# fabriceo/AVDSP

Hardware: AMD Instinct MI355X
Metric: Msamples/s (all ch) biquad+FIR chain (higher is better)
Workload: dtype f64; 1 GPU; north: 4096 ch x (16 biquads + 4096-tap FIR), block 1024 frames, DSP_FORMAT 6; 4096 ch in total, 4096 ch/GPU by dspRuntimeSetShard(rank, 1), no data-path collective; channels=4096, channels_per_gpu=4096, taps=4096, block=1024, format=6, overlap=1, ready_words=-1, ready_mode=2, side_by_side=1, streams_remade=0, cu_split=0, fir_split=0, fir_launch=-1, fir_lean=-1, ring_wait=1

## Files before the change

avdsp_amd/csrc/avdsp_host.c:

```c
#include "avdsp_runtime.h"
#include "avdsp_hip.h"

#include <stdarg.h>
#include <stdio.h>
#include <stdlib.h>
#include <string.h>

dspHeader_t *dspHeaderPtr = 0;
int          dspBiquadFreqSkip = 0;
int          dspMantissa = DSP_MANT;

const char *dspOpcodeText[DSP_MAX_OPCODE] = {
    "DSP_END_OF_CODE", "\nDSP_HEADER", "DSP_NOP", "\nDSP_CORE", "\nDSP_PARAM", "\nDSP_PARAM_NUM",
    "DSP_SERIAL", "DSP_TPDF_CALC", "DSP_TPDF", "DSP_WHITE", "DSP_CLRXY", "DSP_SWAPXY", "DSP_COPYXY",
    "DSP_COPYYX", "DSP_ADDXY", "DSP_ADDYX", "DSP_SUBXY", "DSP_SUBYX", "DSP_MULXY", "DSP_DIVXY",
    "DSP_DIVYX", "DSP_AVGXY", "DSP_AVGYX", "DSP_NEGX", "DSP_NEGY", "DSP_SQRTX", "DSP_SHIFT",
    "DSP_VALUE", "DSP_VALUE_INT", "DSP_MUL_VALUE", "DSP_MUL_VALUE_INT", "DSP_DIV_VALUE",
    "DSP_DIV_VALUE_INT", "DSP_AND_VALUE_INT", "DSP_LOAD", "DSP_LOAD_GAIN", "DSP_LOAD_MUX",
    "DSP_STORE", "DSP_LOAD_STORE", "DSP_LOAD_MEM", "DSP_STORE_MEM", "DSP_GAIN", "DSP_SAT0DB",
    "DSP_SAT0DB_TPDF", "DSP_SAT0DB_GAIN", "DSP_SAT0DB_TPDF_GAIN", "DSP_DELAY_1", "DSP_DELAY",
    "DSP_DELAY_DP", "DSP_DATA_TABLE", "DSP_BIQUADS", "DSP_FIR", "DSP_RMS", "DSP_DCBLOCK",
    "DSP_DITHER", "DSP_DITHER_NS2", "DSP_DISTRIB", "DSP_DIRAC", "DSP_SQUAREWAVE", "DSP_CLIP",
    "DSP_LOAD_MEM_DATA", "DSP_SINE"
};
// ... 52 lines not shown
    int             biquad_freq_skip, mantissa;
    int             device_ordinal;
    int             ninst;
    int             inst_saved_lanes;
    int             inst_saved_generic;
    int             inst_call;
    size_t          inst_in_words, inst_out_words;
    int             opt_cu_split;
    int             opt_group_serial;
    int             inst_chain_mode;
    int             chain_inst_made;
    size_t          chain_inst_in, chain_inst_out;
    int             chain_inst_win[5];
    int             opt_frame_server, opt_frame_server_idle_us;
    int             opt_fir_shared;
} avdsp_ctx;

static avdsp_ctx g_template = { .opt_lane_hw = 1, .opt_ring_wait = 1, .opt_ready_words = -1, .opt_fir_impl = 1, .opt_biquad_impl = 1, .opt_device = -1, .opt_interp_impl = 1, .opt_strand_split = 1, .opt_strand_lanes = 1, .shard_world = 1,
                                .mantissa = DSP_MANT, .device_ordinal = -1, .opt_frame_server_idle_us = 1000, .opt_fir_shared = 1 };

__attribute__((constructor)) static void frame_server_from_environment(void)
{
    const char *e = getenv("AVDSP_FRAME_SERVER");
    if (e && !strcmp(e, "1")) g_template.opt_frame_server = 1;
}
#define MAX_PROGRAMS 64
static avdsp_ctx *g_ctx[MAX_PROGRAMS];
static int        g_nctx;
static avdsp_ctx *g_cur = &g_template;
#define G (*g_cur)
static int        g_rate_static;

static char g_err[512];
static int  g_err_code;
static int  ensure_encoding(int format);

static int fail(int code, const char *fmt, ...)
{
    va_list ap;
// ... 130 lines not shown
        G.opt_host_pin = value;
        return 0;
    }
    if (!strcmp(key, "fir_lean")) {
        if (G.dev && avdsp_hip_prog_set_option(G.dev, AVDSP_OPT_FIR_LEAN, value)) return hip_fail();
        G.opt_fir_lean = value; G.opt_fir_lean_set = 1;
        return 0;
    }
    if (!strcmp(key, "fir_shared")) {
        if (value != 0 && value != 1) return fail(-1, "fir_shared: 0 or 1");
        if (G.dev && avdsp_hip_prog_set_option(G.dev, AVDSP_OPT_FIR_SHARED, value)) return hip_fail();
        G.opt_fir_shared = value;
        return 0;
    }
    if (!strcmp(key, "fir_shared_chains") || !strcmp(key, "fir_shared_groups")) return fail(-1, "%s is read-only", key);
    if (!strcmp(key, "ring_wait")) {
        if (G.dev && avdsp_hip_prog_set_option(G.dev, AVDSP_OPT_RING_WAIT, value)) return hip_fail();
        G.opt_ring_wait = value != 0;
        return 0;
    }
    if (!strcmp(key, "fir_launch")) {
        if (G.dev && avdsp_hip_prog_set_option(G.dev, AVDSP_OPT_FIR_LAUNCH, value)) return hip_fail();
        G.opt_fir_launch = value; G.opt_fir_launch_set = 1;
        return 0;
    }
    if (!strcmp(key, "profile_stride")) {
        if (value < 1) return fail(-1, "profile_stride: every n-th launch, n >= 1");
        if (G.dev && avdsp_hip_prog_set_option(G.dev, AVDSP_OPT_PROFILE_STRIDE, value)) return hip_fail();
        G.opt_profile_stride = value;
        return 0;
// ... 59 lines not shown
    if (!strcmp(key, "interp_impl")) return G.opt_interp_impl;
    if (!strcmp(key, "levels"))      return G.last_levels;
    if (!strcmp(key, "cores"))       return G.last_cores;
    if (!strcmp(key, "pieces"))      return G.last_pieces;
    if (!strcmp(key, "strand_split")) return G.opt_strand_split;
    if (!strcmp(key, "strand_lanes")) return G.opt_strand_lanes;
    if (!strcmp(key, "strands"))     return G.last_strands;
    if (!strcmp(key, "overlap"))     return G.opt_overlap;
    if (!strcmp(key, "ready_words")) return G.opt_ready_words;
    if (!strcmp(key, "lane_hw"))     return G.opt_lane_hw;
    if (!strcmp(key, "fir_split"))   return G.opt_fir_split;
    if (!strcmp(key, "fir_launch"))  return G.opt_fir_launch_set ? G.opt_fir_launch : -1;
    if (!strcmp(key, "fir_lean"))    return G.opt_fir_lean_set ? G.opt_fir_lean : -1;
    if (!strcmp(key, "ring_wait"))   return G.opt_ring_wait;
    if (!strcmp(key, "fir_shared"))  return G.opt_fir_shared;
    if (!strcmp(key, "fir_shared_chains")) { device_current(); return G.dev ? avdsp_hip_prog_get_option(G.dev, AVDSP_OPT_FIR_SHARED_CHAINS) : 0; }
    if (!strcmp(key, "fir_shared_groups")) { device_current(); return G.dev ? avdsp_hip_prog_get_option(G.dev, AVDSP_OPT_FIR_SHARED_GROUPS) : 0; }
    if (!strncmp(key, "timing_pairs_", 13) && key[13] >= '0' && key[13] <= '7' && !key[14])
        return G.dev ? avdsp_hip_profile_last_pairs(G.dev, key[13] - '0') : 0;
    if (!strcmp(key, "ready_timeouts")) { device_current(); return G.dev ? avdsp_hip_ready_timeouts(G.dev) : 0; }
    if (!strcmp(key, "cu_split"))    return G.opt_cu_split;
    if (!strcmp(key, "group_fanout")) return !G.opt_group_serial;
    if (!strcmp(key, "side_by_side")) { device_current(); return G.dev ? avdsp_hip_prog_get_option(G.dev, AVDSP_OPT_SIDE_BY_SIDE) : -1; }
    if (!strcmp(key, "streams_remade")) { device_current(); return G.dev ? avdsp_hip_prog_get_option(G.dev, AVDSP_OPT_STREAMS_REMADE) : 0; }
    if (!strcmp(key, "ready_mode"))  { device_current(); return G.dev ? avdsp_hip_prog_get_option(G.dev, AVDSP_OPT_READY_MODE) : 0; }
    if (!strcmp(key, "frame_server")) return G.opt_frame_server;
    if (!strcmp(key, "frame_server_idle_us")) return G.opt_frame_server_idle_us;
    if (!strcmp(key, "frame_server_frames")) return G.dev ? avdsp_hip_prog_get_option(G.dev, AVDSP_OPT_FRAME_SERVER_FRAMES) : 0;
    if (!strcmp(key, "frame_server_launches")) return G.dev ? avdsp_hip_prog_get_option(G.dev, AVDSP_OPT_FRAME_SERVER_LAUNCHES) : 0;
    if (!strcmp(key, "frame_server_fallbacks")) return G.dev ? avdsp_hip_prog_get_option(G.dev, AVDSP_OPT_FRAME_SERVER_FALLBACKS) : 0;
// ... 91 lines not shown
        const dspHeader_t *h = (const dspHeader_t *)codePtr;
        const opcode_t *lo = codePtr, *hi = codePtr + (long long)h->totalLength + (h->dataSize > 0 ? h->dataSize : 0);
        for (int i = 0; i < g_nctx; )
            if (g_ctx[i] != c && g_ctx[i]->code < hi && lo < g_ctx[i]->code + (g_ctx[i]->total_words > 0 ? g_ctx[i]->total_words : 1)) ctx_destroy(g_ctx[i]);
            else i++;
    }
    int fresh = 0;
    if (!c) {
        if (g_nctx == MAX_PROGRAMS) return fail(-9, "%d programs are loaded already: dspRuntimeReleaseProgram() the ones no longer used", MAX_PROGRAMS);
        c = (avdsp_ctx *)calloc(1, sizeof *c);
        if (!c) return fail(-9, "out of memory");
        const avdsp_ctx *o = &g_template;
        c->opt_fir_impl = o->opt_fir_impl; c->opt_biquad_impl = o->opt_biquad_impl; c->opt_device = o->opt_device; c->opt_profile = o->opt_profile;
        c->opt_generic = o->opt_generic; c->opt_interp_impl = o->opt_interp_impl; c->opt_strand_split = o->opt_strand_split; c->opt_strand_lanes = o->opt_strand_lanes;
        c->opt_profile_stride = o->opt_profile_stride; c->opt_overlap = o->opt_overlap; c->opt_fir_rows = o->opt_fir_rows; c->opt_host_split = o->opt_host_split; c->opt_host_pin = o->opt_host_pin; c->opt_ready_words = o->opt_ready_words; c->opt_lane_hw = o->opt_lane_hw; c->opt_fir_split = o->opt_fir_split; c->opt_fir_launch = o->opt_fir_launch; c->opt_fir_launch_set = o->opt_fir_launch_set; c->opt_fir_lean = o->opt_fir_lean; c->opt_fir_lean_set = o->opt_fir_lean_set; c->opt_ring_wait = o->opt_ring_wait; c->opt_cu_split = o->opt_cu_split; c->opt_group_serial = o->opt_group_serial;
        c->opt_frame_server = o->opt_frame_server; c->opt_frame_server_idle_us = o->opt_frame_server_idle_us; c->opt_fir_shared = o->opt_fir_shared;
        c->shard_rank = o->shard_rank; c->shard_world = o->shard_world;
        c->mantissa = DSP_MANT; c->device_ordinal = -1;
        c->code = codePtr;
        g_ctx[g_nctx++] = c;
        fresh = 1;
    }
    ctx_make_current(c);
    drop_device();
    G.have_rate = 0;
    dspHeaderPtr = (dspHeader_t *)codePtr;
    G.code = codePtr;
    G.total_words = 0;
#define INIT_FAIL(...) do { const int r_ = fail(__VA_ARGS__); if (fresh) { ctx_destroy(c); for (int i_ = 0; i_ < g_nctx; i_++) if (g_ctx[i_] == prev) ctx_make_current(prev); } return r_; } while (0)
    if (codePtr->op.opcode != DSP_HEADER) INIT_FAIL(-1, "no dsp header in this program");
    int length = dspHeaderPtr->totalLength, size = dspHeaderPtr->dataSize;
// ... 698 lines not shown
    if (!G.dev) return hip_fail();
    if (avdsp_hip_upload_words(G.dev, (const int32_t *)G.code, 0, G.total_words) ||
        avdsp_hip_tpdf_reset(G.dev, G.random, G.dither)) {
        hip_fail(); drop_device(); return g_err_code;
    }
    G.dev_state_valid = 1;
    avdsp_hip_profile_enable(G.dev, G.opt_profile);
    if (avdsp_hip_prog_set_option(G.dev, AVDSP_OPT_PROFILE_STRIDE, G.opt_profile_stride > 0 ? G.opt_profile_stride : 1) ||
        avdsp_hip_prog_set_option(G.dev, AVDSP_OPT_OVERLAP, G.opt_overlap) || avdsp_hip_prog_set_option(G.dev, AVDSP_OPT_FIR_ROWS, G.opt_fir_rows) ||
        avdsp_hip_prog_set_option(G.dev, AVDSP_OPT_READY_WORDS, G.opt_ready_words) || avdsp_hip_prog_set_option(G.dev, AVDSP_OPT_LANE_HW, G.opt_lane_hw) || avdsp_hip_prog_set_option(G.dev, AVDSP_OPT_FIR_SPLIT, G.opt_fir_split) || (G.opt_fir_launch_set && avdsp_hip_prog_set_option(G.dev, AVDSP_OPT_FIR_LAUNCH, G.opt_fir_launch)) || (G.opt_fir_lean_set && avdsp_hip_prog_set_option(G.dev, AVDSP_OPT_FIR_LEAN, G.opt_fir_lean)) || avdsp_hip_prog_set_option(G.dev, AVDSP_OPT_RING_WAIT, G.opt_ring_wait) ||
        avdsp_hip_prog_set_option(G.dev, AVDSP_OPT_HOST_SPLIT, G.opt_host_split) || avdsp_hip_prog_set_option(G.dev, AVDSP_OPT_HOST_PIN, G.opt_host_pin) ||
        (G.opt_cu_split && avdsp_hip_prog_set_option(G.dev, AVDSP_OPT_CU_SPLIT, G.opt_cu_split)) ||
        (G.opt_group_serial && avdsp_hip_prog_set_option(G.dev, AVDSP_OPT_GROUP_FANOUT, 0)) ||
        (G.opt_frame_server && avdsp_hip_prog_set_option(G.dev, AVDSP_OPT_FRAME_SERVER, 1)) ||
        (!G.opt_fir_shared && avdsp_hip_prog_set_option(G.dev, AVDSP_OPT_FIR_SHARED, 0)) ||
        (G.opt_frame_server_idle_us != 1000 && avdsp_hip_prog_set_option(G.dev, AVDSP_OPT_FRAME_SERVER_IDLE_US, G.opt_frame_server_idle_us)) ||
        (G.ninst > 1 && avdsp_hip_set_instances(G.dev, G.ninst))) {
        hip_fail(); drop_device(); return g_err_code;
    }
    return 0;
}

static const avdsp_chain *g_fg_chains;
static int fir_group_cmp(const void *pa, const void *pb)
{
    const avdsp_chain *a = &g_fg_chains[*(const int32_t *)pa], *b = &g_fg_chains[*(const int32_t *)pb];
    if (a->fir_coef_word != b->fir_coef_word) return a->fir_coef_word < b->fir_coef_word ? -1 : 1;
    if (a->fir_taps != b->fir_taps) return a->fir_taps < b->fir_taps ? -1 : 1;
    return *(const int32_t *)pa < *(const int32_t *)pb ? -1 : *(const int32_t *)pa > *(const int32_t *)pb;
}
// ... 1179 lines not shown
```

avdsp_amd/csrc/avdsp_kernels.hip:

```cpp
#include <hip/hip_runtime.h>
#include <hip/hip_ext.h>
#include <atomic>
#include <chrono>
#include <mutex>
#include <thread>

#include <cstdarg>
#include <cstdio>
#include <cstring>
#include <type_traits>
#include <utility>
#include <vector>
#include <algorithm>

#include "avdsp_hip.h"
#include "avdsp_format.h"

namespace {

thread_local char g_err[512];
thread_local bool g_err_ready = false;

int set_err(const char *fmt, ...)
{
// ... 3213 lines not shown
    double *d_taps64 = nullptr; int pitch64 = 0;
    int n_sh_groups = 0, n_sh_chains = 0;
    int *d_sh_ids = nullptr;
    SharedTile *d_sh_tiles = nullptr; int n_sh_tiles = 0;
    double *d_sh_taps64 = nullptr;
    int *d_sh_feed = nullptr; int n_sh_feed = 0;
    int *d_fir_rest = nullptr; int n_fir_rest = 0;
    bool lane_mode = false;
    int *d_lane_rows = nullptr; int n_lane_rows = 0;
    int n_lane_feed = 0;
    int n_lane_fir = 0; unsigned *d_lseq = nullptr; int lseq_pitch = 0;
    avdsp_strand_op *d_sops = nullptr; int *d_sargs = nullptr; int s_nops = 0, s_nargs = 0, s_nstrands = 0, s_nres = 0; bool s_usey = false;
    std::vector<int> s_loaded, s_stored;
    bool stores_whole_window = false;
    bool overlap_ok = false;
    unsigned *d_ready = nullptr; unsigned seq = 0;
};

}

struct avdsp_hip_prog {
    int total_words = 0;
    int chain_inst = 0;
    int *d_buf = nullptr;
    TpdfGlobals *d_tpdf = nullptr;
    int *d_tpdf_seq = nullptr; int tpdf_seq_frames = 0;
    unsigned *d_frame = nullptr; int frame_words = 0;
    std::vector<Plan> plans;
    unsigned *d_in = nullptr, *d_out = nullptr; size_t in_cap = 0, out_cap = 0;
    struct Alias { hipStream_t stream; unsigned *buf; size_t cap; };
// ... 21 lines not shown
    std::vector<hipStream_t> side;
    std::vector<hipEvent_t> join;
    hipEvent_t fork = nullptr;
    int overlap = 0;
    int fir_rows = 0;
    int fir_lean = -1;
    int fir_split = 0;
    int fir_shared = 1;
    int sh_chains_now = 0, sh_groups_now = 0;
    hipStream_t s_bq = nullptr;
    hipStream_t s_fir[2] = {nullptr, nullptr};
    static constexpr int kAhead = 3;
    hipEvent_t ev_bq[kAhead] = {nullptr, nullptr, nullptr}, ev_fir[kAhead] = {nullptr, nullptr, nullptr};
    hipEvent_t ev_fir_now[kAhead] = {nullptr, nullptr, nullptr};
    hipEvent_t last_ride_stop = nullptr;
    int fir_launch_mode = -1, fir_mode_now = 0;
    hipEvent_t launch_ev[16] = {};
    unsigned launch_ev_next = 0;
    int lane_hw = 1;
    int ready_words = -1;
    int ready_mode_now = 0;
    int side_by_side = 0;
    std::vector<std::pair<hipStream_t, int>> probed;
    std::vector<hipStream_t> retired;
    int remade = 0;
    hipStream_t bq_side[3] = {nullptr, nullptr, nullptr};
    hipEvent_t bq_fork = nullptr, bq_join[3] = {nullptr, nullptr, nullptr};
    int group_fanout = 1;
    int cu_split = 0;
    unsigned *d_ready_timeouts = nullptr;
// ... 117 lines not shown
    if (v.empty()) return 0;
    HIP_TRY(hipMalloc((void **)dst, v.size() * sizeof(T)));
    return copy_from_caller(*dst, v.data(), v.size() * sizeof(T));
}

void free_plan(Plan &p)
{
    (void)hipFree(p.d_chains); (void)hipFree(p.d_sec_coef); (void)hipFree(p.d_sec_state);
    for (auto &g : p.bq) {
        (void)hipFree(g.d_ids); (void)hipFree(g.d_rows); (void)hipFree(g.d_lanes); (void)hipFree(g.d_scratch[0]); (void)hipFree(g.d_scratch[1]);
        for (auto &pc : g.pieces) { (void)hipFree(pc.d_ids); (void)hipFree(pc.d_rows); (void)hipFree(pc.d_lanes); }
    }
    (void)hipFree(p.d_rows_all); (void)hipFree(p.d_lanes_all);
    (void)hipFree(p.d_sops); (void)hipFree(p.d_sargs); (void)hipFree(p.d_lseq); (void)hipFree(p.d_lane_rows);
    (void)hipFree(p.d_fir_ids); (void)hipFree(p.d_pass_ids); (void)hipFree(p.d_ring); (void)hipFree(p.d_ring64); (void)hipFree(p.d_own); (void)hipFree(p.d_taps64);
    (void)hipFree(p.d_ready);
    (void)hipFree(p.d_sh_ids); (void)hipFree(p.d_sh_tiles); (void)hipFree(p.d_sh_taps64); (void)hipFree(p.d_sh_feed); (void)hipFree(p.d_fir_rest);
}

int fir_groups_per_chunk(int max_taps)
{
    const int G = (max_taps + 15 + 15) >> 4;
    const int nc = (G + kMaxGpc - 1) / kMaxGpc;
    const int gpc = (G + nc - 1) / nc;
    return std::min((gpc + kNG - 1) / kNG * kNG, kMaxGpc);
}

size_t fir_lds_bytes(int gpc, int *hs_cap, int *row)
{
    *hs_cap = (fir_hs_len(gpc) + 3) & ~3;
    *row = fir_win_row(gpc);
// ... 477 lines not shown
    HIP_TRY(hipEventRecord(prog->bq_fork, st));
    for (int k = 1; k < lanes; k++) HIP_TRY(hipStreamWaitEvent(prog->bq_side[k - 1], prog->bq_fork, 0));
    for (size_t gi = 0; gi < ng; gi++) {
        auto &g = *todo[gi];
        const int k = (int)(gi % (size_t)lanes);
        if (launch_group(g, k ? prog->bq_side[k - 1] : st, nullptr)) return -1;
    }
    for (int k = 1; k < lanes; k++) {
        HIP_TRY(hipEventRecord(prog->bq_join[k - 1], prog->bq_side[k - 1]));
        HIP_TRY(hipStreamWaitEvent(st, prog->bq_join[k - 1], 0));
    }
    if (last_stop) HIP_TRY(hipEventRecord(last_stop, st));
    return 0;
}

template <int FMT>
int launch_all(avdsp_hip_prog *prog, Plan &pl, BlockIO io, int fir_impl, int biquad_impl, hipStream_t stream)
{
    const bool under = prog->overlap && pl.overlap_ok && biquad_impl && fir_impl;
    pl.seq++;
    if (under) {
        prog->sh_chains_now = prog->sh_groups_now = 0;
        if (overlap_ready(prog)) return -1;
        const bool own_fir = prog->overlap >= 2 || prog->cu_split > 0;
        if (probe_side_by_side(prog, prog->overlap >= 2 ? prog->s_fir[prog->blk & 1] : prog->cu_split > 0 ? prog->s_fir[0] : stream)) return -1;
        const bool can_words = (fir_impl == 1 || fir_impl == 4) && pl.d_ready && prog->d_ready_timeouts && prog->side_by_side;
        const int rw = prog->ready_words >= 0 ? prog->ready_words : (prog->overlap == 1 && (long long)pl.n_fir * pl.max_taps >= 12000000ll ? 2 : 0);
        const bool behind = rw == 2 && can_words;
        const bool words = (rw == 1 && fir_impl == 1 && can_words) || behind;
        prog->ready_mode_now = behind ? 2 : words ? 1 : 0;
        const bool wt = words && !behind;
        const int slot = (int)(prog->blk % avdsp_hip_prog::kAhead);
        if (prog->ev_fir_set[slot]) {
            bool done = false;
            if (prog->ring_wait_host) {
                const auto t0 = std::chrono::steady_clock::now();
                for (;;) {
                    const hipError_t q = hipEventQuery(prog->ev_fir_now[slot]);
                    if (q == hipSuccess) { done = true; break; }
                    (void)hipGetLastError();
                    if (q != hipErrorNotReady) break;
                    if (std::chrono::steady_clock::now() - t0 > std::chrono::milliseconds(1)) break;
                    std::this_thread::yield();
                }
            }
            if (!done) HIP_TRY(hipStreamWaitEvent(prog->s_bq, prog->ev_fir_now[slot], 0));
        }
        if (prog->input_ready) HIP_TRY(hipStreamWaitEvent(prog->s_bq, prog->input_ready, 0));
        if (launch_cascades<FMT>(prog, pl, io, biquad_impl, prog->s_bq, !words ? prog->ev_bq[slot] : nullptr, wt)) return -1;
        if (behind && prog->ready_test > 0) prog->ready_test--;
        else if (behind) {
            hipLaunchKernelGGL(ready_set, dim3((unsigned)((pl.n_fir + kBlock - 1) / kBlock)), dim3(kBlock), 0, prog->s_bq, pl.d_ready, pl.d_fir_ids, pl.n_fir, pl.seq);
            HIP_TRY(hipGetLastError());
        }
        if (own_fir) {
            hipStream_t fs = prog->s_fir[prog->overlap >= 2 ? (prog->blk & 1) : 0];
            if (!words) HIP_TRY(hipStreamWaitEvent(fs, prog->ev_bq[slot], 0));
            if (launch_fir<FMT>(prog, pl, pl.d_fir_ids, pl.n_fir, io, fir_impl, fs, words)) return -1;
            HIP_TRY(hipEventRecord(prog->ev_fir[slot], fs));
            prog->ev_fir_now[slot] = prog->ev_fir[slot];
            HIP_TRY(hipStreamWaitEvent(stream, prog->ev_fir[slot], 0));
        } else {
            if (!words) HIP_TRY(hipStreamWaitEvent(stream, prog->ev_bq[slot], 0));
            const int mode = fir_impl != 1 && fir_impl != 4 ? 0 : prog->fir_launch_mode >= 0 ? prog->fir_launch_mode
                           : ((long long)pl.n_fir * pl.max_taps <= 6000000ll && io.nframes > 768) ? 2 : 1;
            const bool rides = mode == 1 && !((prog->profile >> AVDSP_KERNEL_FIR & 1u) && prog->profile_seen[AVDSP_KERNEL_FIR & 7] % (unsigned)prog->profile_stride == 0);
            prog->fir_mode_now = mode;
            prog->last_ride_stop = nullptr;
            const int rc_fir = launch_fir<FMT>(prog, pl, pl.d_fir_ids, pl.n_fir, io, fir_impl, stream, words, rides ? prog->ev_fir[slot] : nullptr);
            prog->fir_mode_now = 0;
            if (rc_fir) return -1;
            prog->ev_fir_now[slot] = prog->ev_fir[slot];
            static const bool timer_doubles = !getenv("AVDSP_TIMER_DOUBLES") || atoi(getenv("AVDSP_TIMER_DOUBLES")) != 0;
            if (!rides && mode == 1 && prog->last_ride_stop && timer_doubles) prog->ev_fir_now[slot] = prog->last_ride_stop;
            else if (!rides) HIP_TRY(hipEventRecord(prog->ev_fir[slot], stream));
        }
// ... 254 lines not shown
    (void)hipFree(p->d_tag_prev);
    for (auto &pn : p->pinned) if (pn.ours) (void)hipHostUnregister(const_cast<void *>(pn.ptr));
    for (auto st : {p->s_h2d, p->s_run, p->s_d2h}) if (st) (void)hipStreamDestroy(st);
    for (auto e : p->ev_host) (void)hipEventDestroy(e);
    for (auto st : {p->q_h2d, p->q_run, p->q_d2h}) if (st) { (void)hipStreamSynchronize(st); (void)hipStreamDestroy(st); }
    for (auto &sl : p->hq) {
        (void)hipFree(sl.d_in); (void)hipFree(sl.d_out);
        for (auto e : {sl.h2d, sl.run, sl.d2h}) if (e) (void)hipEventDestroy(e);
    }
    if (p->s_bq) (void)hipStreamDestroy(p->s_bq);
    for (auto st : p->retired) (void)hipStreamDestroy(st);
    for (auto st : p->bq_side) if (st) (void)hipStreamDestroy(st);
    for (auto e : p->bq_join) if (e) (void)hipEventDestroy(e);
    if (p->bq_fork) (void)hipEventDestroy(p->bq_fork);
    for (auto fs : p->s_fir) if (fs) (void)hipStreamDestroy(fs);
    if (p->ev_unpack) (void)hipEventDestroy(p->ev_unpack);
    for (int i = 0; i < avdsp_hip_prog::kAhead; i++) { if (p->ev_bq[i]) (void)hipEventDestroy(p->ev_bq[i]); if (p->ev_fir[i]) (void)hipEventDestroy(p->ev_fir[i]); }
    (void)hipFree(p->d_buf); (void)hipFree(p->d_in); (void)hipFree(p->d_out); (void)hipFree(p->d_tpdf); (void)hipFree(p->d_frame);
    (void)hipHostFree(p->h_small); (void)hipHostFree(p->h_ready_flag);
    (void)hipHostFree(p->fs_h); (void)hipFree(p->fs_table);
    for (auto e : p->launch_ev) if (e) (void)hipEventDestroy(e);
    (void)hipFree(p->d_tpdf_seq); (void)hipFree(p->d_ready_timeouts); for (auto &x : p->alias) (void)hipFree(x.buf);
    (void)hipFree(p->d_inst_buf); (void)hipFree(p->d_inst_tpdf); (void)hipFree(p->d_inst_frame); (void)hipFree(p->d_inst_seq);
    delete p;
}

int avdsp_hip_prog_add_plan(avdsp_hip_prog *prog, const avdsp_plan_desc *d)
{
    FS_STOP(prog);
    if (d->format < 2 || d->format > 6) return set_err("format %d has no device kernels", d->format);
// ... 115 lines not shown
            while (all_rows.size() % 4) { all_rows.push_back(empty); all_lanes.insert(all_lanes.end(), 16, LaneRec{-1, -1}); }
            pl.n_row_groups++;
            pl.rows_all_fir = pl.rows_all_fir && all_fir;
        }
        pl.bq.push_back(g);
    }
    if (upload_vec(&pl.d_chains, dev_chains)) { free_plan(pl); return -1; }
    if (pl.n_row_groups >= 2) {
        RowRec empty = all_rows.back(); empty.cid = -1;
        while (all_rows.size() % 16) { all_rows.push_back(empty); all_lanes.insert(all_lanes.end(), 16, LaneRec{-1, -1}); }
        pl.n_rows_all = (int)all_rows.size();
        if (upload_vec(&pl.d_rows_all, all_rows) || upload_vec(&pl.d_lanes_all, all_lanes)) { free_plan(pl); return -1; }
    }
    pl.n_fir = (int)fir.size(); pl.n_pass = (int)pass.size();
    if (upload_vec(&pl.d_fir_ids, fir) || upload_vec(&pl.d_pass_ids, pass)) { free_plan(pl); return -1; }
    if (pl.n_fir) {
        pl.fir_gpc = fir_groups_per_chunk(pl.max_taps);
        {
            int hs_cap, row;
            const int lds = (int)fir_lds_bytes(pl.fir_gpc, &hs_cap, &row);
            const void *variants[2] = { d->format == 4 ? (const void *)fir_mfma<4, 1> : (const void *)fir_mfma<6, 1>,
                                        d->format == 4 ? (const void *)fir_mfma<4, 2> : (const void *)fir_mfma<6, 2> };
            for (const void *fn : variants) {
                hipError_t e = hipFuncSetAttribute(fn, hipFuncAttributeMaxDynamicSharedMemorySize, lds);
                if (e != hipSuccess) { free_plan(pl); return set_err("hipFuncSetAttribute(LDS %d): %s", lds, hipGetErrorString(e)); }
            }
        }
        pl.ring_R = pow2ceil(pl.max_taps + avdsp_hip_prog::kAhead * kFirChunk + 16 * pl.fir_gpc + 16 * (kNG + 4) + 64);
        static_assert(kFirChunk == kFirPad, "one FIR launch covers exactly the frames the window image is laid out for");
        hipError_t e = hipMalloc((void **)&pl.d_ring, (size_t)d->nchains * 2 * pl.ring_R * sizeof(float));
// ... 1328 lines not shown
    (void)hipFree(d);
    return rc;
}

int avdsp_hip_prog_set_option(avdsp_hip_prog *prog, int key, int value)
{
    FS_STOP(prog);
    HIP_TRY(hipDeviceSynchronize());
    switch (key) {
    case AVDSP_OPT_OVERLAP:  prog->overlap = value; for (bool &f : prog->ev_fir_set) f = false; return 0;
    case AVDSP_OPT_READY_WORDS: if (value < -1 || value > 2) return set_err("ready_words: -1 (by plan), 0 (events), 1 (the cascade's waves publish) or 2 (a kernel behind the cascade publishes)"); prog->ready_words = value; return 0;
    case AVDSP_OPT_LANE_HW: prog->lane_hw = value != 0; return 0;
    case AVDSP_OPT_FIR_SPLIT: prog->fir_split = value != 0; return 0;
    case AVDSP_OPT_FIR_SHARED: if (value != 0 && value != 1) return set_err("fir_shared: 0 or 1"); prog->fir_shared = value; return 0;
    case AVDSP_OPT_FIR_LEAN: if (value < -1 || value > 1) return set_err("fir_lean: -1 (auto), 0 or 1"); prog->fir_lean = value; return 0;
    case AVDSP_OPT_RING_WAIT: prog->ring_wait_host = value != 0; return 0;
    case AVDSP_OPT_READY_TEST: prog->ready_test = value > 0 ? value : 0; return 0;
    case AVDSP_OPT_FRAME_SERVER: prog->fs_on = value != 0; return 0;
    case AVDSP_OPT_FRAME_SERVER_IDLE_US: if (value < 50 || value > 20000) return set_err("frame_server_idle_us: 50 .. 20000"); prog->fs_idle_us = value; return 0;
    case AVDSP_OPT_GROUP_FANOUT: prog->group_fanout = value != 0; return 0;
    case AVDSP_OPT_CU_SPLIT:
        if (value < -128 || value > 128 || (value & 7)) return set_err("cu_split: 0 (off) or 8, 16, ... 128 CUs for the cascades' stream (negative: the FIRs stay on the caller's stream, unmasked)");
        if (value != prog->cu_split) {
            if (prog->s_bq) { (void)hipStreamDestroy(prog->s_bq); prog->s_bq = nullptr; }
            for (auto &fs : prog->s_fir) if (fs) { (void)hipStreamDestroy(fs); fs = nullptr; }
            for (int i = 0; i < avdsp_hip_prog::kAhead; i++) {
                if (prog->ev_bq[i]) { (void)hipEventDestroy(prog->ev_bq[i]); prog->ev_bq[i] = nullptr; }
                if (prog->ev_fir[i]) { (void)hipEventDestroy(prog->ev_fir[i]); prog->ev_fir[i] = nullptr; }
                prog->ev_fir_set[i] = false; prog->ev_fir_now[i] = nullptr;
            }
// ... 19 lines not shown

int avdsp_hip_prog_get_option(avdsp_hip_prog *prog, int key)
{
    switch (key) {
    case AVDSP_OPT_SIDE_BY_SIDE: return prog->s_bq ? prog->side_by_side : -1;
    case AVDSP_OPT_READY_MODE:   return prog->ready_mode_now;
    case AVDSP_OPT_STREAMS_REMADE: return prog->remade;
    case AVDSP_OPT_FRAME_SERVER: return prog->fs_on;
    case AVDSP_OPT_FRAME_SERVER_IDLE_US: return prog->fs_idle_us;
    case AVDSP_OPT_FRAME_SERVER_FRAMES: return (int)std::min(prog->fs_frames, 0x7FFFFFFFll);
    case AVDSP_OPT_FRAME_SERVER_LAUNCHES: return (int)std::min(prog->fs_launches, 0x7FFFFFFFll);
    case AVDSP_OPT_FRAME_SERVER_FALLBACKS: return (int)std::min(prog->fs_fallbacks, 0x7FFFFFFFll);
    case AVDSP_OPT_FIR_SHARED: return prog->fir_shared;
    case AVDSP_OPT_FIR_SHARED_CHAINS: return prog->sh_chains_now;
    case AVDSP_OPT_FIR_SHARED_GROUPS: return prog->sh_groups_now;
    }
    return -1;
}

int avdsp_hip_ready_clear(avdsp_hip_prog *prog)
{
    FS_STOP(prog);
    if (!prog->d_ready_timeouts) return 0;
    HIP_TRY(hipDeviceSynchronize());
    HIP_TRY(hipMemset(prog->d_ready_timeouts, 0, 4));
    if (prog->h_ready_flag) *(volatile unsigned *)prog->h_ready_flag = 0;
    return 0;
}

int avdsp_hip_last_error_is_ready_timeout(void) { return g_err_ready ? 1 : 0; }
// ... 49 lines not shown
```

include/avdsp_hip.h:

```cpp
#ifndef AVDSP_HIP_H_
#define AVDSP_HIP_H_

#include <stddef.h>
#include <stdint.h>

#ifdef __cplusplus
extern "C" {
#endif

#define AVDSP_MAX_STORES 4

enum { AVDSP_LOAD_PLAIN = 0, AVDSP_LOAD_GAIN = 1 };

typedef struct avdsp_chain {
    int32_t  in_io;
    int32_t  load_mode;
    uint32_t gain_bits;
    int32_t  nsec;
    int32_t  sec_base;
    int32_t  fir_taps;
    int32_t  fir_coef_word;
    int32_t  fir_state_word;
    int32_t  sat;
    int32_t  n_out;
// ... 125 lines not shown
enum { AVDSP_OPT_OVERLAP = 0, AVDSP_OPT_PROFILE_STRIDE = 1, AVDSP_OPT_FIR_ROWS = 3, AVDSP_OPT_HOST_SPLIT = 4, AVDSP_OPT_HOST_PIN = 5,
       AVDSP_OPT_READY_WORDS = 6, AVDSP_OPT_LANE_HW = 7, AVDSP_OPT_FIR_SPLIT = 8, AVDSP_OPT_FIR_LAUNCH = 9, AVDSP_OPT_FIR_LEAN = 10, AVDSP_OPT_RING_WAIT = 11,
       AVDSP_OPT_SIDE_BY_SIDE = 13,
       AVDSP_OPT_GROUP_FANOUT = 17,
       AVDSP_OPT_CU_SPLIT = 16,
       AVDSP_OPT_STREAMS_REMADE = 15,
       AVDSP_OPT_READY_MODE = 14,
       AVDSP_OPT_READY_TEST = 12,
       AVDSP_OPT_FRAME_SERVER = 18,
       AVDSP_OPT_FRAME_SERVER_IDLE_US = 19,
       AVDSP_OPT_FRAME_SERVER_FRAMES = 20,
       AVDSP_OPT_FRAME_SERVER_LAUNCHES = 21,
       AVDSP_OPT_FRAME_SERVER_FALLBACKS = 22,
       AVDSP_OPT_FIR_SHARED = 23,
       AVDSP_OPT_FIR_SHARED_CHAINS = 24,
       AVDSP_OPT_FIR_SHARED_GROUPS = 25          };
int avdsp_hip_chain_instances(avdsp_hip_prog *prog, int n);
int avdsp_hip_prog_get_option(avdsp_hip_prog *prog, int key);
int avdsp_hip_ready_clear(avdsp_hip_prog *prog);
int avdsp_hip_last_error_is_ready_timeout(void);
int avdsp_hip_ready_timeouts(avdsp_hip_prog *prog);
int avdsp_hip_prog_set_option(avdsp_hip_prog *prog, int key, int value);

int avdsp_hip_tag_output(avdsp_hip_prog *prog, void *d_column, int stride, int nframes, int reset, int reset_value, void *stream);

int avdsp_hip_tag_column_host(avdsp_hip_prog *prog, int *h_column, int nframes);

int avdsp_hip_synchronize(void *stream);
const char *avdsp_hip_last_error(void);

#ifdef __cplusplus
// ... 4 lines not shown
```

Before: 8457 Msamples/s.

## Run large FIR on alternating streams into staging buffers, then copy to output

Adds a FIR-alternate mode, chosen by default for large FIR plans (n_fir*taps above a threshold). In this mode the FIR runs on a per-block alternating stream and writes into per-slot staging buffers, and a small copy kernel on the main stream then scatters the results into the output. This replaces the ready-word handshake so consecutive blocks' FIR work can overlap without a write conflict on the shared output. The cost is an extra device copy pass, more event waits and three staging buffers.

```diff
diff --git a/avdsp_amd/csrc/avdsp_host.c b/avdsp_amd/csrc/avdsp_host.c
--- a/avdsp_amd/csrc/avdsp_host.c
+++ b/avdsp_amd/csrc/avdsp_host.c
@@ -90,15 +90,18 @@
     int             chain_inst_win[5];
     int             opt_frame_server, opt_frame_server_idle_us;
     int             opt_fir_shared;
+    int             opt_fir_alternate;
 } avdsp_ctx;
 
 static avdsp_ctx g_template = { .opt_lane_hw = 1, .opt_ring_wait = 1, .opt_ready_words = -1, .opt_fir_impl = 1, .opt_biquad_impl = 1, .opt_device = -1, .opt_interp_impl = 1, .opt_strand_split = 1, .opt_strand_lanes = 1, .shard_world = 1,
-                                .mantissa = DSP_MANT, .device_ordinal = -1, .opt_frame_server_idle_us = 1000, .opt_fir_shared = 1 };
+                                .mantissa = DSP_MANT, .device_ordinal = -1, .opt_frame_server_idle_us = 1000, .opt_fir_shared = 1, .opt_fir_alternate = -1 };
 
 __attribute__((constructor)) static void frame_server_from_environment(void)
 {
     const char *e = getenv("AVDSP_FRAME_SERVER");
     if (e && !strcmp(e, "1")) g_template.opt_frame_server = 1;
+    e = getenv("AVDSP_FIR_ALTERNATE");
+    if (e && (!strcmp(e, "-1") || !strcmp(e, "0") || !strcmp(e, "1"))) g_template.opt_fir_alternate = atoi(e);
 }
 #define MAX_PROGRAMS 64
 static avdsp_ctx *g_ctx[MAX_PROGRAMS];
@@ -259,6 +262,13 @@
         return 0;
     }
     if (!strcmp(key, "fir_shared_chains") || !strcmp(key, "fir_shared_groups")) return fail(-1, "%s is read-only", key);
+    if (!strcmp(key, "fir_alternate")) {
+        if (value < -1 || value > 1) return fail(-1, "fir_alternate: -1 (by plan), 0 or 1");
+        if (G.dev && avdsp_hip_prog_set_option(G.dev, AVDSP_OPT_FIR_ALTERNATE, value)) return hip_fail();
+        G.opt_fir_alternate = value;
+        return 0;
+    }
+    if (!strcmp(key, "fir_alternate_now")) return fail(-1, "%s is read-only", key);
     if (!strcmp(key, "ring_wait")) {
         if (G.dev && avdsp_hip_prog_set_option(G.dev, AVDSP_OPT_RING_WAIT, value)) return hip_fail();
         G.opt_ring_wait = value != 0;
@@ -348,6 +358,8 @@
     if (!strcmp(key, "fir_lean"))    return G.opt_fir_lean_set ? G.opt_fir_lean : -1;
     if (!strcmp(key, "ring_wait"))   return G.opt_ring_wait;
     if (!strcmp(key, "fir_shared"))  return G.opt_fir_shared;
+    if (!strcmp(key, "fir_alternate")) return G.opt_fir_alternate;
+    if (!strcmp(key, "fir_alternate_now")) { device_current(); return G.dev ? avdsp_hip_prog_get_option(G.dev, AVDSP_OPT_FIR_ALTERNATE_NOW) : 0; }
     if (!strcmp(key, "fir_shared_chains")) { device_current(); return G.dev ? avdsp_hip_prog_get_option(G.dev, AVDSP_OPT_FIR_SHARED_CHAINS) : 0; }
     if (!strcmp(key, "fir_shared_groups")) { device_current(); return G.dev ? avdsp_hip_prog_get_option(G.dev, AVDSP_OPT_FIR_SHARED_GROUPS) : 0; }
     if (!strncmp(key, "timing_pairs_", 13) && key[13] >= '0' && key[13] <= '7' && !key[14])
@@ -469,7 +481,7 @@
         c->opt_fir_impl = o->opt_fir_impl; c->opt_biquad_impl = o->opt_biquad_impl; c->opt_device = o->opt_device; c->opt_profile = o->opt_profile;
         c->opt_generic = o->opt_generic; c->opt_interp_impl = o->opt_interp_impl; c->opt_strand_split = o->opt_strand_split; c->opt_strand_lanes = o->opt_strand_lanes;
         c->opt_profile_stride = o->opt_profile_stride; c->opt_overlap = o->opt_overlap; c->opt_fir_rows = o->opt_fir_rows; c->opt_host_split = o->opt_host_split; c->opt_host_pin = o->opt_host_pin; c->opt_ready_words = o->opt_ready_words; c->opt_lane_hw = o->opt_lane_hw; c->opt_fir_split = o->opt_fir_split; c->opt_fir_launch = o->opt_fir_launch; c->opt_fir_launch_set = o->opt_fir_launch_set; c->opt_fir_lean = o->opt_fir_lean; c->opt_fir_lean_set = o->opt_fir_lean_set; c->opt_ring_wait = o->opt_ring_wait; c->opt_cu_split = o->opt_cu_split; c->opt_group_serial = o->opt_group_serial;
-        c->opt_frame_server = o->opt_frame_server; c->opt_frame_server_idle_us = o->opt_frame_server_idle_us; c->opt_fir_shared = o->opt_fir_shared;
+        c->opt_frame_server = o->opt_frame_server; c->opt_frame_server_idle_us = o->opt_frame_server_idle_us; c->opt_fir_shared = o->opt_fir_shared; c->opt_fir_alternate = o->opt_fir_alternate;
         c->shard_rank = o->shard_rank; c->shard_world = o->shard_world;
         c->mantissa = DSP_MANT; c->device_ordinal = -1;
         c->code = codePtr;
@@ -1198,6 +1210,7 @@
         (G.opt_group_serial && avdsp_hip_prog_set_option(G.dev, AVDSP_OPT_GROUP_FANOUT, 0)) ||
         (G.opt_frame_server && avdsp_hip_prog_set_option(G.dev, AVDSP_OPT_FRAME_SERVER, 1)) ||
         (!G.opt_fir_shared && avdsp_hip_prog_set_option(G.dev, AVDSP_OPT_FIR_SHARED, 0)) ||
+        (G.opt_fir_alternate != -1 && avdsp_hip_prog_set_option(G.dev, AVDSP_OPT_FIR_ALTERNATE, G.opt_fir_alternate)) ||
         (G.opt_frame_server_idle_us != 1000 && avdsp_hip_prog_set_option(G.dev, AVDSP_OPT_FRAME_SERVER_IDLE_US, G.opt_frame_server_idle_us)) ||
         (G.ninst > 1 && avdsp_hip_set_instances(G.dev, G.ninst))) {
         hip_fail(); drop_device(); return g_err_code;
diff --git a/avdsp_amd/csrc/avdsp_kernels.hip b/avdsp_amd/csrc/avdsp_kernels.hip
--- a/avdsp_amd/csrc/avdsp_kernels.hip
+++ b/avdsp_amd/csrc/avdsp_kernels.hip
@@ -3251,6 +3251,7 @@
     std::vector<int> s_loaded, s_stored;
     bool stores_whole_window = false;
     bool overlap_ok = false;
+    int *d_fir_cols = nullptr; int n_fir_cols = 0, fir_col_lo = 0, fir_col_hi = -1; bool fir_cols_run = false;
     unsigned *d_ready = nullptr; unsigned seq = 0;
 };
 
@@ -3302,6 +3303,9 @@
     hipEvent_t ev_bq[kAhead] = {nullptr, nullptr, nullptr}, ev_fir[kAhead] = {nullptr, nullptr, nullptr};
     hipEvent_t ev_fir_now[kAhead] = {nullptr, nullptr, nullptr};
     hipEvent_t last_ride_stop = nullptr;
+    int fir_alternate = -1, fir_alternate_now = 0;
+    unsigned *d_stage[kAhead] = {nullptr, nullptr, nullptr}; size_t stage_cap = 0;
+    hipEvent_t ev_done[kAhead] = {nullptr, nullptr, nullptr};
     int fir_launch_mode = -1, fir_mode_now = 0;
     hipEvent_t launch_ev[16] = {};
     unsigned launch_ev_next = 0;
@@ -3449,7 +3453,7 @@
     (void)hipFree(p.d_rows_all); (void)hipFree(p.d_lanes_all);
     (void)hipFree(p.d_sops); (void)hipFree(p.d_sargs); (void)hipFree(p.d_lseq); (void)hipFree(p.d_lane_rows);
     (void)hipFree(p.d_fir_ids); (void)hipFree(p.d_pass_ids); (void)hipFree(p.d_ring); (void)hipFree(p.d_ring64); (void)hipFree(p.d_own); (void)hipFree(p.d_taps64);
-    (void)hipFree(p.d_ready);
+    (void)hipFree(p.d_ready); (void)hipFree(p.d_fir_cols);
     (void)hipFree(p.d_sh_ids); (void)hipFree(p.d_sh_tiles); (void)hipFree(p.d_sh_taps64); (void)hipFree(p.d_sh_feed); (void)hipFree(p.d_fir_rest);
 }
 
@@ -3957,18 +3961,74 @@
     return 0;
 }
 
+struct OutCopyArgs {
+    const unsigned *src; unsigned *dst;
+    int src_stride, src_base, dst_stride, dst_base;
+    int nframes, lo, n4;
+    const int *cols; int ncols;
+};
+
+__global__ __launch_bounds__(256) void out_copy(const OutCopyArgs a)
+{
+    const long long step = (long long)gridDim.x * blockDim.x;
+    long long i = (long long)blockIdx.x * blockDim.x + threadIdx.x;
+    if (!a.cols) {
+        const long long total = (long long)a.nframes * a.n4;
+        for (; i < total; i += step) {
+            const int f = (int)(i / a.n4), p = (int)(i - (long long)f * a.n4);
+            const uint4 v = *reinterpret_cast<const uint4 *>(a.src + (size_t)f * a.src_stride + (a.lo - a.src_base) + 4 * p);
+            *reinterpret_cast<uint4 *>(a.dst + (size_t)f * a.dst_stride + (a.lo - a.dst_base) + 4 * p) = v;
+        }
+    } else {
+        const long long total = (long long)a.nframes * a.ncols;
+        for (; i < total; i += step) {
+            const int f = (int)(i / a.ncols), io = a.cols[(int)(i - (long long)f * a.ncols)];
+            a.dst[(size_t)f * a.dst_stride + (io - a.dst_base)] = a.src[(size_t)f * a.src_stride + (io - a.src_base)];
+        }
+    }
+}
+
+static bool stage_ready(avdsp_hip_prog *prog, size_t words)
+{
+    for (auto &e : prog->ev_done)
+        if (!e && hipEventCreateWithFlags(&e, hipEventDisableTiming | hipEventDisableSystemFence) != hipSuccess) { (void)hipGetLastError(); e = nullptr; return false; }
+    if (words <= prog->stage_cap) return true;
+    if (hipDeviceSynchronize() != hipSuccess) return false;
+    for (auto &b : prog->d_stage) { (void)hipFree(b); b = nullptr; }
+    prog->stage_cap = 0;
+    for (auto &b : prog->d_stage)
+        if (hipMalloc((void **)&b, words * sizeof(unsigned)) != hipSuccess) {
+            (void)hipGetLastError();
+            for (auto &x : prog->d_stage) { (void)hipFree(x); x = nullptr; }
+            return false;
+        }
+    prog->stage_cap = words;
+    return true;
+}
+
 template <int FMT>
 int launch_all(avdsp_hip_prog *prog, Plan &pl, BlockIO io, int fir_impl, int biquad_impl, hipStream_t stream)
 {
     const bool under = prog->overlap && pl.overlap_ok && biquad_impl && fir_impl;
     pl.seq++;
+    prog->fir_alternate_now = 0;
     if (under) {
         prog->sh_chains_now = prog->sh_groups_now = 0;
         if (overlap_ready(prog)) return -1;
-        const bool own_fir = prog->overlap >= 2 || prog->cu_split > 0;
-        if (probe_side_by_side(prog, prog->overlap >= 2 ? prog->s_fir[prog->blk & 1] : prog->cu_split > 0 ? prog->s_fir[0] : stream)) return -1;
+        bool alt = prog->overlap == 1 && prog->fir_alternate != 0 && fir_impl == 1 && prog->cu_split == 0 && !prog->fir_split && pl.instances <= 1 &&
+                   prog->ready_words <= 0 && pl.n_fir_cols > 0 && io.out_stride > 0;
+        if (alt && prog->fir_alternate < 0) alt = (long long)pl.n_fir * pl.max_taps >= 12000000ll;
+        if (alt) {
+            const char *i0 = (const char *)io.in, *i1 = i0 + (size_t)io.nframes * io.in_stride * 4;
+            const char *o0 = (const char *)io.out, *o1 = o0 + (size_t)io.nframes * io.out_stride * 4;
+            if (i0 < o1 && o0 < i1) alt = false;
+        }
+        const int st_base = io.out_base + ((pl.fir_col_lo - io.out_base) & ~3), st_pitch = (pl.fir_col_hi - st_base + 1 + 3) & ~3;
+        if (alt && (pl.fir_col_lo < io.out_base || !stage_ready(prog, (size_t)kFirChunk * st_pitch))) alt = false;
+        const bool own_fir = alt || prog->overlap >= 2 || prog->cu_split > 0;
+        if (probe_side_by_side(prog, alt || prog->overlap >= 2 ? prog->s_fir[prog->blk & 1] : prog->cu_split > 0 ? prog->s_fir[0] : stream)) return -1;
         const bool can_words = (fir_impl == 1 || fir_impl == 4) && pl.d_ready && prog->d_ready_timeouts && prog->side_by_side;
-        const int rw = prog->ready_words >= 0 ? prog->ready_words : (prog->overlap == 1 && (long long)pl.n_fir * pl.max_taps >= 12000000ll ? 2 : 0);
+        const int rw = alt ? 0 : prog->ready_words >= 0 ? prog->ready_words : (prog->overlap == 1 && (long long)pl.n_fir * pl.max_taps >= 12000000ll ? 2 : 0);
         const bool behind = rw == 2 && can_words;
         const bool words = (rw == 1 && fir_impl == 1 && can_words) || behind;
         prog->ready_mode_now = behind ? 2 : words ? 1 : 0;
@@ -3988,6 +4048,7 @@
                 }
             }
             if (!done) HIP_TRY(hipStreamWaitEvent(prog->s_bq, prog->ev_fir_now[slot], 0));
+            if (!done && alt) HIP_TRY(hipStreamWaitEvent(prog->s_fir[prog->blk & 1], prog->ev_fir_now[slot], 0));
         }
         if (prog->input_ready) HIP_TRY(hipStreamWaitEvent(prog->s_bq, prog->input_ready, 0));
         if (launch_cascades<FMT>(prog, pl, io, biquad_impl, prog->s_bq, !words ? prog->ev_bq[slot] : nullptr, wt)) return -1;
@@ -3997,12 +4058,42 @@
             HIP_TRY(hipGetLastError());
         }
         if (own_fir) {
-            hipStream_t fs = prog->s_fir[prog->overlap >= 2 ? (prog->blk & 1) : 0];
+            hipStream_t fs = prog->s_fir[alt || prog->overlap >= 2 ? (prog->blk & 1) : 0];
             if (!words) HIP_TRY(hipStreamWaitEvent(fs, prog->ev_bq[slot], 0));
-            if (launch_fir<FMT>(prog, pl, pl.d_fir_ids, pl.n_fir, io, fir_impl, fs, words)) return -1;
+            BlockIO fio = io;
+            if (alt) {
+                if (prog->input_ready && pl.n_fir_only) HIP_TRY(hipStreamWaitEvent(fs, prog->input_ready, 0));
+                const int prev = (slot + avdsp_hip_prog::kAhead - 1) % avdsp_hip_prog::kAhead;
+                if (pl.n_fir_only && prog->ev_fir_set[prev])
+                    HIP_TRY(hipStreamWaitEvent(fs, prog->ev_fir_now[prev] == prog->ev_done[prev] ? prog->ev_fir[prev] : prog->ev_fir_now[prev], 0));
+                fio.out = prog->d_stage[slot]; fio.out_stride = st_pitch; fio.out_base = st_base;
+            }
+            if (launch_fir<FMT>(prog, pl, pl.d_fir_ids, pl.n_fir, fio, fir_impl, fs, words)) return -1;
             HIP_TRY(hipEventRecord(prog->ev_fir[slot], fs));
             prog->ev_fir_now[slot] = prog->ev_fir[slot];
             HIP_TRY(hipStreamWaitEvent(stream, prog->ev_fir[slot], 0));
+            if (alt) {
+                OutCopyArgs ca{};
+                ca.src = fio.out; ca.src_stride = st_pitch; ca.src_base = st_base;
+                ca.dst = io.out;  ca.dst_stride = io.out_stride; ca.dst_base = io.out_base;
+                ca.nframes = io.nframes; ca.lo = pl.fir_col_lo;
+                const int ncol = pl.fir_col_hi - pl.fir_col_lo + 1;
+                const bool pieces = pl.fir_cols_run && !(ncol & 3) && !((pl.fir_col_lo - io.out_base) & 3) && !(io.out_stride & 3) &&
+                                    !(reinterpret_cast<size_t>(io.out) & 15);
+                long long total;
+                if (pieces) { ca.n4 = ncol / 4; total = (long long)io.nframes * ca.n4; }
+                else        { ca.cols = pl.d_fir_cols; ca.ncols = pl.n_fir_cols; total = (long long)io.nframes * ca.ncols; }
+#ifndef AVDSP_NO_OUT_COPY
+                const int per = pieces ? 4 : 8;
+                hipLaunchKernelGGL(out_copy, dim3((unsigned)std::min<long long>((total + 256 * per - 1) / (256 * per), 4096)), dim3(256), 0, stream, ca);
+                HIP_TRY(hipGetLastError());
+#else
+                (void)total;
+#endif
+                HIP_TRY(hipEventRecord(prog->ev_done[slot], stream));
+                prog->ev_fir_now[slot] = prog->ev_done[slot];
+                prog->fir_alternate_now = 1;
+            }
         } else {
             if (!words) HIP_TRY(hipStreamWaitEvent(stream, prog->ev_bq[slot], 0));
             const int mode = fir_impl != 1 && fir_impl != 4 ? 0 : prog->fir_launch_mode >= 0 ? prog->fir_launch_mode
@@ -4287,6 +4378,8 @@
     for (auto e : p->bq_join) if (e) (void)hipEventDestroy(e);
     if (p->bq_fork) (void)hipEventDestroy(p->bq_fork);
     for (auto fs : p->s_fir) if (fs) (void)hipStreamDestroy(fs);
+    for (auto b : p->d_stage) (void)hipFree(b);
+    for (auto e : p->ev_done) if (e) (void)hipEventDestroy(e);
     if (p->ev_unpack) (void)hipEventDestroy(p->ev_unpack);
     for (int i = 0; i < avdsp_hip_prog::kAhead; i++) { if (p->ev_bq[i]) (void)hipEventDestroy(p->ev_bq[i]); if (p->ev_fir[i]) (void)hipEventDestroy(p->ev_fir[i]); }
     (void)hipFree(p->d_buf); (void)hipFree(p->d_in); (void)hipFree(p->d_out); (void)hipFree(p->d_tpdf); (void)hipFree(p->d_frame);
@@ -4432,6 +4525,18 @@
     }
     pl.n_fir = (int)fir.size(); pl.n_pass = (int)pass.size();
     if (upload_vec(&pl.d_fir_ids, fir) || upload_vec(&pl.d_pass_ids, pass)) { free_plan(pl); return -1; }
+    if (pl.n_fir) {
+        std::vector<int> cols;
+        for (int id : fir) for (int k = 0; k < chains[id].n_out; k++) cols.push_back(chains[id].out_io[k]);
+        pl.n_fir_cols = (int)cols.size();
+        pl.fir_col_lo = *std::min_element(cols.begin(), cols.end()); pl.fir_col_hi = *std::max_element(cols.begin(), cols.end());
+        {
+            std::vector<int> u = cols;
+            std::sort(u.begin(), u.end());
+            pl.fir_cols_run = std::adjacent_find(u.begin(), u.end()) == u.end() && (long long)pl.fir_col_hi - pl.fir_col_lo + 1 == (long long)u.size();
+        }
+        if (upload_vec(&pl.d_fir_cols, cols)) { free_plan(pl); return -1; }
+    }
     if (pl.n_fir) {
         pl.fir_gpc = fir_groups_per_chunk(pl.max_taps);
         {
@@ -5790,6 +5895,7 @@
     case AVDSP_OPT_FIR_SPLIT: prog->fir_split = value != 0; return 0;
     case AVDSP_OPT_FIR_SHARED: if (value != 0 && value != 1) return set_err("fir_shared: 0 or 1"); prog->fir_shared = value; return 0;
     case AVDSP_OPT_FIR_LEAN: if (value < -1 || value > 1) return set_err("fir_lean: -1 (auto), 0 or 1"); prog->fir_lean = value; return 0;
+    case AVDSP_OPT_FIR_ALTERNATE: if (value < -1 || value > 1) return set_err("fir_alternate: -1 (by plan), 0 or 1"); prog->fir_alternate = value; return 0;
     case AVDSP_OPT_RING_WAIT: prog->ring_wait_host = value != 0; return 0;
     case AVDSP_OPT_READY_TEST: prog->ready_test = value > 0 ? value : 0; return 0;
     case AVDSP_OPT_FRAME_SERVER: prog->fs_on = value != 0; return 0;
@@ -5839,6 +5945,8 @@
     case AVDSP_OPT_FIR_SHARED: return prog->fir_shared;
     case AVDSP_OPT_FIR_SHARED_CHAINS: return prog->sh_chains_now;
     case AVDSP_OPT_FIR_SHARED_GROUPS: return prog->sh_groups_now;
+    case AVDSP_OPT_FIR_ALTERNATE: return prog->fir_alternate;
+    case AVDSP_OPT_FIR_ALTERNATE_NOW: return prog->fir_alternate_now;
     }
     return -1;
 }
diff --git a/include/avdsp_hip.h b/include/avdsp_hip.h
--- a/include/avdsp_hip.h
+++ b/include/avdsp_hip.h
@@ -163,7 +163,9 @@
        AVDSP_OPT_FRAME_SERVER_FALLBACKS = 22,
        AVDSP_OPT_FIR_SHARED = 23,
        AVDSP_OPT_FIR_SHARED_CHAINS = 24,
-       AVDSP_OPT_FIR_SHARED_GROUPS = 25          };
+       AVDSP_OPT_FIR_SHARED_GROUPS = 25,
+       AVDSP_OPT_FIR_ALTERNATE = 26,
+       AVDSP_OPT_FIR_ALTERNATE_NOW = 27          };
 int avdsp_hip_chain_instances(avdsp_hip_prog *prog, int n);
 int avdsp_hip_prog_get_option(avdsp_hip_prog *prog, int key);
 int avdsp_hip_ready_clear(avdsp_hip_prog *prog);
```

After: 8247 Msamples/s. 2.5% lower.
